# widkyyu/Goal-conditioned-Reinforcement-Learning-with-environmental-and-policy-priors

Measured on AMD Instinct MI355X. Metric: env-steps/sec, higher is better.
Workload: dtype u8

## Files before the change

### goal-conditioned-reinforcement-learning-with-environmental-and-policy-priors_amd/_lib.py

```python
import ctypes as C
import os
import subprocess

_PKG_DIR = os.path.dirname(os.path.abspath(__file__))
LIB_PATH = os.path.join(_PKG_DIR, "libtwoarmy_hip.so")
CSRC_DIR = os.path.join(_PKG_DIR, "csrc")

TW_CELLS = 289
TW_REC_WORDS = 48
TW_DRAW_WORDS = 8
TW_F_AUTORESET = 1
TW_F_POLICY_IDX = 2
TW_F_MATRIX_CODE = 4
TW_F_SLAB_HIPMALLOC = 8

FIELDS = dict(AX=0, AY=1, DIR=2, STEP_COUNT=3, STEP_MOVE=4, PONE=5, PATROL=6, UP1=7, RIGHT2=8, UPD_LONG=9,
              UPD_HORIZ=10, RISK=11, FIRST_ROOM2=12, OBX=13, OBY=16, O1X=19, O1Y=22, O1_VALID=25, O2X=26,
              O2Y=30, O2_VALID=34, GOAL_X=35, GOAL_Y=36, T=37, ERROR=38, MAX_STEPS=39, EPISODES=40,
              LAST_REWARD=41, LAST_TERM=42, LAST_TRUNC=43, WALL_I1=44, WALL_I2=45)

LAUNCH_FIELDS = ("pipelined", "PG", "LAYOUT", "pipe_grid", "E", "FAST", "seq_grid", "T")

ENV_ERRORS = {1: AttributeError, 2: AssertionError, 3: TypeError}

# ... 77 lines not shown
    "mg_obs_goal_direction": (C.c_int, [_vp, _i, _i, _i, _vp, _vp, _i, _i, _vp, _vp, _vp, _vp]),
    "mg_nav_field": (C.c_int, [_vp, _vp, _i, _i, _i, C.c_uint32, _i, _vp, _vp, _i, _vp, _vp, _i, _vp, _i64, _vp, _vp, _vp,
                               _vp]),
    "mg_nav_lookup": (C.c_int, [_vp, _i64, _i, _i, _i, _vp, _i, _vp, _vp]),
    "mg_nav_optimal_moves": (C.c_int, [_vp, _i64, _i, _i, _i, _vp, _vp, _vp, _i, _vp, _vp, _vp]),
    "mg_nav_goal_moves": (C.c_int, [_vp, _vp, _i, _i, _i, C.c_uint32, _i, _vp, _vp, _vp, _i64, _vp, _vp, _vp, _i, _vp, _vp,
                                    _vp]),
    "mg_nav_timed_field": (C.c_int, [_vp, _vp, _i, _i, _i, C.c_uint32, _i, _vp, _i64, _i, _vp, _vp, _i, _vp, _vp, _vp, _i, _vp,
                                     _i64, _vp, _vp, _vp, _vp]),
    "mg_nav_timed_moves": (C.c_int, [_vp, _i64, _i, _i, _i, _i, _vp, _vp, _vp, _i, _vp, _vp, _vp]),
    "mg_nav_timed_goal_moves": (C.c_int, [_vp, _vp, _i, _i, _i, C.c_uint32, _i, _vp, _i64, _i, _vp, _vp, _vp, _i64, _vp, _vp,
                                          _vp, _i, _vp, _vp, _vp]),
    "mg_nav_timed_goal_floods": (C.c_int, [_i, _i, _i]),
    "mg_nav_shape": (C.c_int, [_vp, _i64, _i, _i, _i, _i, _vp, _vp, _vp, _vp, _vp, _vp, _i, _f, _f, _i, _vp, _vp, _vp, _vp]),
    "mg_nav_goal_shape": (C.c_int, [_vp, _vp, _i, _i, _i, C.c_uint32, _i, _vp, _vp, _vp, _vp, _vp, _i64, _vp, _vp, _vp, _vp,
                                    _i, _f, _f, _vp, _vp, _vp, _vp]),
    "mg_nav_timed_goal_shape": (C.c_int, [_vp, _vp, _i, _i, _i, C.c_uint32, _i, _vp, _i64, _i, _vp, _vp, _vp, _vp, _vp, _i64,
                                          _vp, _vp, _vp, _vp, _i, _f, _f, _vp, _vp, _vp, _vp]),
    "mg_nav_timed_goal_shape_floods": (C.c_int, [_i, _i, _i]),
    "mg_nav_ahead": (C.c_int, [_vp, _i64, _i, _i, _i, _i, _vp, _vp, _vp, _i, _i, _vp, _vp, _vp]),
    "mg_nav_goal_ahead": (C.c_int, [_vp, _vp, _i, _i, _i, C.c_uint32, _i, _vp, _vp, _vp, _i64, _vp, _vp, _vp, _i, _i, _vp,
                                    _vp, _vp]),
    "mg_nav_timed_goal_ahead": (C.c_int, [_vp, _vp, _i, _i, _i, C.c_uint32, _i, _vp, _i64, _i, _vp, _vp, _vp, _i64, _vp, _vp,
                                          _vp, _i, _i, _vp, _vp, _vp]),
    "mg_nav_timed_goal_ahead_floods": (C.c_int, [_i, _i, _i]),
    "mg_nav_path_scan": (C.c_int, [_vp, _i64, _i, _i, _i, _i, _vp, _vp, _vp, _vp, _vp, _vp, _i, _vp, _vp, _vp, _vp, _vp, _vp,
                                   _vp, _vp, _vp]),
    "mg_nav_path_summary_workspace": (C.c_int, [_i, _i]),
    "mg_nav_path_summary": (C.c_int, [_vp, _vp, _vp, _vp, _vp, _vp, _i, _i, _vp, _vp, _vp]),
    "ppo_her_relabel": (C.c_int, [_vp, _vp, _vp, _vp, _vp, _vp, _u64, C.c_uint32, C.c_uint32, _i, _i, _i, _vp, _vp, _vp,
                                  _vp, _vp, _vp, _vp, _vp]),
    "ppo_her_relabel_window": (C.c_int, [_vp, _vp, _vp, _vp, _vp, _vp, _u64, C.c_uint32, C.c_uint32, _i, _i, _i, _i, _vp,
                                         _vp, _vp, _vp, _vp, _vp, _vp, _vp]),
    "ppo_lstm_cell": (C.c_int, [_vp, _vp, C.c_longlong, _vp, _vp, _vp, _i, _i, _vp]),
    "ppo_decoder_frames": (C.c_int, [_vp, _i, _vp, _vp, _vp, _vp, _vp, C.c_float, _vp, _vp]),
    "ppo_gather_stack_u8": (C.c_int, [_vp, _i, _vp, _i, _vp, _vp, _vp, _vp, _vp, _i, _vp, _vp, _vp]),
    "ppo_age_scan": (C.c_int, [_vp, _vp, _vp, _i, _i, _vp, _vp]),
    "ppo_episode_scan": (C.c_int, [_vp, _vp, _vp, _i, _i, _vp, _vp, _vp, _vp, _vp]),
    "ppo_episode_summary": (C.c_int, [_vp, _vp, _vp, _vp, _vp, _vp, _i, _i, _i, C.c_double, C.c_double, _vp, _vp, _vp, _vp,
                                      _vp, _vp]),
    "ppo_episode_summary_workspace": (C.c_int, [_i, _i]),
    "ppo_visit_scan": (C.c_int, [_vp, _vp, _vp, _i, _i, _i, _i, _vp, _vp, _vp, _vp]),
    "ppo_visit_carry_words": (C.c_int, [_i, _i, _i]),
    "ppo_visit_hist": (C.c_int, [_vp, _i, _i, _vp, _vp, _vp, _i, _i, _i, _vp, _vp]),
    "ppo_bonus_table_words": (C.c_int, [_i, _i, _i, _i, _i, _i]),
    "ppo_bonus_workspace_bytes": (_i64, [_i, _i, _i, _i, _i, _i]),
    "ppo_bonus_scan": (C.c_int, [_vp, _vp, _vp, C.c_long, C.c_long, _vp, _vp, _i, _i, _i, _i, _i, _i, _i, C.c_double, _vp, _vp,
                                 _vp, _vp, _vp, _vp, _vp]),
    "ppo_bias_relu_nhwc": (C.c_int, [_vp, _vp, _i64, _i, _vp]),
    "ppo_conv1_up4_bias_relu": (C.c_int, [_vp, _i, _i, _vp, _vp, _vp, _vp]),
    "ppo_conv1_up4_bias_relu_c": (C.c_int, [_vp, _i, _i, _i, _vp, _vp, _vp, _vp]),
    "ppo_conv1_up4_bwd_groups": (C.c_int, [_i]),
    "ppo_conv1_up4_bwd": (C.c_int, [_vp, _i, _i, _vp, _vp, _vp, _vp, _vp]),
    "ppo_relu_bwd_bias_grad_nhwc_blocks": (C.c_int, [_i64, _i]),
    "ppo_relu_bwd_bias_grad_nhwc": (C.c_int, [_vp, _vp, _vp, _vp, _i64, _i, _vp]),
})

_lib = None


def exported_symbols():
    return sorted(_SIGS)


def lib():
    global _lib
    if _lib is None:
        if not os.path.exists(LIB_PATH):
            raise TwoarmyLibraryError(
                "%s not built: run `python -c 'import __graft_entry__ as g; g.build()'` "
                "(hipcc --offload-arch=gfx950); there is no CPU fallback" % LIB_PATH)
        import torch
        try:
            h = C.CDLL(LIB_PATH)
        except OSError as ex:
            raise TwoarmyLibraryError("cannot load %s: %s" % (LIB_PATH, ex)) from ex
        for name, (res, args) in _SIGS.items():
            try:
                fn = getattr(h, name)
            except AttributeError as ex:
                raise TwoarmyLibraryError("%s lacks symbol %s" % (LIB_PATH, name)) from ex
            fn.restype, fn.argtypes = res, args
        runtimes = set()
        try:
            with open("/proc/self/maps") as f:
                for line in f:
                    if "libamdhip64" in line:
                        runtimes.add(line.split()[-1])
        except OSError:
            pass
        if h.tw_abi_sizeof_outputs() != C.sizeof(TwOutputs):
            raise TwoarmyLibraryError("struct tw_outputs: the library has %d bytes, the ctypes mirror %d"
                                      % (h.tw_abi_sizeof_outputs(), C.sizeof(TwOutputs)))
        if len(runtimes) > 1:
            raise TwoarmyLibraryError("two HIP runtimes mapped (%s): import torch before loading %s"
                                      % (sorted(runtimes), LIB_PATH))
        _lib = h
    return _lib


def check(rc, what):
    if rc != 0:
        raise TwoarmyLibraryError("%s failed: rc=%d hipError=%d %s" % (
            what, rc, lib().tw_last_hip_error(), lib().tw_last_error_message().decode()))
```

### goal-conditioned-reinforcement-learning-with-environmental-and-policy-priors_amd/csrc/ppo_kernels.hip

```cpp

#include <hip/hip_runtime.h>
#include <float.h>
#include <stdint.h>

#include <type_traits>

#include "launch.h"
#include "philox.h"
#include "twoarmy.h"
#include "twoarmy_ppo.h"

namespace {

constexpr float CAT_EPS = FLT_EPSILON;

template <int A> __device__ __forceinline__ float cat_row(const float *__restrict__ row, float (&p)[A]) {
    float S = 0.f;
#pragma unroll
    for (int k = 0; k < A; ++k) { p[k] = row[k]; S += p[k]; }
    return S;
}
__device__ __forceinline__ float cat_log(float q) { return logf(fminf(fmaxf(q, CAT_EPS), 1.0f - CAT_EPS)); }

template <typename T, int K> __device__ __forceinline__ void block_sum(T (&v)[K], T *lds) {
// ... 131 lines not shown
            float4 acc = bv;
#pragma unroll
            for (int t = 0; t < 4; ++t) {
                const int ty = t >> 1, tx = t & 1;
#pragma unroll
                for (int c = 0; c < F; ++c) acc = fma4(xs[c * 324 + (m + ty) * 18 + n + tx], w[t * F + c], acc);
            }
            dst[((2 * m + py) * 33 + 2 * n + px) * CQ + cq] = relu4(acc);
        }
    }
}

template <int F>
__global__ __launch_bounds__(256) void ppo_conv1_up4_bwd_kernel(const float *__restrict__ frames, const float4 *__restrict__ gy,
                                                                const float4 *__restrict__ y, float4 *__restrict__ gw_part,
                                                                float4 *__restrict__ gb_part, int B) {
    __shared__ float xs[F * 18 * 18];
    __shared__ float4 red[256];
    const int tid = threadIdx.x, cq = tid & 15, slot = tid >> 4;
    const int ph = blockIdx.y, py = ph >> 1, px = ph & 1;
    const int ny = 17 - py, nx = 17 - px;
    float4 acc[4 * F];
#pragma unroll
    for (int k = 0; k < 4 * F; ++k) acc[k] = make_float4(0.f, 0.f, 0.f, 0.f);
    float4 accb = make_float4(0.f, 0.f, 0.f, 0.f);
    for (int b = blockIdx.x; b < B; b += gridDim.x) {
        __syncthreads();
        conv1_stage_frame<F>(xs, frames + (size_t)b * F * 289, tid);
        __syncthreads();
        const size_t base = (size_t)b * 1089 * 16;
        for (int q = slot; q < ny * nx; q += 16) {
            const int m = q / nx, n = q - m * nx;
            const size_t o = base + (size_t)((2 * m + py) * 33 + 2 * n + px) * 16 + cq;
            const float4 g = mask4(gy[o], y[o]);
            add4(accb, g);
#pragma unroll
            for (int t = 0; t < 4; ++t) {
                const int ty = t >> 1, tx = t & 1;
#pragma unroll
                for (int c = 0; c < F; ++c) acc[t * F + c] = fma4(xs[c * 324 + (m + ty) * 18 + n + tx], g, acc[t * F + c]);
            }
        }
    }
    const size_t wbase = ((size_t)blockIdx.x * 4 + ph) * (4 * F) * 16;
#pragma unroll
    for (int k = 0; k <= 4 * F; ++k) {
        __syncthreads();
        red[tid] = k < 4 * F ? acc[k < 4 * F ? k : 0] : accb;
        __syncthreads();
        if (slot == 0) {
            const float4 sum = slot_sum4(red, 16, 16, cq);
            if (k < 4 * F) gw_part[wbase + (size_t)k * 16 + cq] = sum;
            else gb_part[((size_t)blockIdx.x * 4 + ph) * 16 + cq] = sum;
        }
    }
}

constexpr int GT = 64;

template <int GN>
__global__ __launch_bounds__(256) void ppo_gae_kernel(const float *__restrict__ reward, const float *__restrict__ value,
                                                      const float *__restrict__ next_value,
                                                      const uint8_t *__restrict__ done, float gamma, float lambda,
                                                      int use_done_mask, int T, int N, float *__restrict__ adv,
                                                      float *__restrict__ target, float *__restrict__ ret) {
    __shared__ float sd[GT][GN + 1];
    __shared__ float sc[GT][GN + 1];
    __shared__ float carry[GN];
    constexpr int ROWS = 256 / GN;
    const int tid = threadIdx.x, tx = tid % GN, ty = tid / GN;
    const int n = blockIdx.x * GN + tx;
    if (tid < GN) carry[tid] = 0.f;
    const int nchunks = (T + GT - 1) / GT;
    for (int ch = nchunks - 1; ch >= 0; --ch) {
        const int t0 = ch * GT;
        __syncthreads();
        for (int r = ty; r < GT; r += ROWS) {
            const int t = t0 + r;
            float d = 0.f, c = 1.f;
            if (t < T && n < N) {
                const size_t i = (size_t)t * N + n;
                const float cut = (use_done_mask && done[i]) ? 0.f : 1.f;
                const float tv = reward[i] + (gamma * next_value[i]) * cut;
                if (target) target[i] = tv;
                d = tv - value[i];
                c = gamma * lambda * cut;
            }
            sd[r][tx] = d; sc[r][tx] = c;
        }
        __syncthreads();
        const int wave = tid >> 6, lane = tid & 63;
        for (int e = wave * (GN / 4); e < (wave + 1) * (GN / 4); ++e) {
            float d = sd[lane][e], c = sc[lane][e];
#pragma unroll
            for (int off = 1; off < 64; off <<= 1) {
                const float d2 = __shfl_down(d, off), c2 = __shfl_down(c, off);
                if (lane + off < 64 && c != 0.f) { d = fmaf(c, d2, d); c = c * c2; }
            }
            const float a = c != 0.f ? fmaf(c, carry[e], d) : d;
            sd[lane][e] = a;
            const float a0 = __shfl(a, 0);
            if (lane == 0) carry[e] = a0;
        }
        __syncthreads();
        for (int r = ty; r < GT; r += ROWS) {
            const int t = t0 + r;
            if (t < T && n < N) {
                const size_t i = (size_t)t * N + n;
// ... 705 lines not shown
                    const float4 *a = reinterpret_cast<const float4 *>(&a2s[(iy * 33 + ix) * 16]);
                    const float4 *k = reinterpret_cast<const float4 *>(&Ks[(u * 3 + v) * 16]);
#pragma unroll
                    for (int c = 0; c < 4; ++c) {
                        const float4 av = a[c], kv = k[c];
                        acc = fmaf(av.x, kv.x, acc); acc = fmaf(av.y, kv.y, acc);
                        acc = fmaf(av.z, kv.z, acc); acc = fmaf(av.w, kv.w, acc);
                    }
                }
            }
            frames[(size_t)f * 289 + o] = acc;
        }
    }
}

__global__ __launch_bounds__(256) void ppo_lstm_cell_kernel(const float4 *__restrict__ ga, const float4 *__restrict__ gb,
                                                            long long ldb4, const float4 *__restrict__ bias,
                                                            float4 *__restrict__ c, float4 *__restrict__ h, int B, int H4) {
    const int i = blockIdx.x * 256 + threadIdx.x;
    if (i >= B * H4) return;
    const int b = i / H4, j = i - b * H4;
    float4 gi = make_float4(0.f, 0.f, 0.f, 0.f), gf = gi, gg = gi, go = gi;
    if (ga) {
        const float4 *g = ga + (size_t)b * 4 * H4;
        gi = g[j]; gf = g[H4 + j]; gg = g[2 * H4 + j]; go = g[3 * H4 + j];
    }
    auto add4 = [](float4 &a, const float4 &v) { a.x += v.x; a.y += v.y; a.z += v.z; a.w += v.w; };
    if (gb) {
        const float4 *q = gb + (size_t)b * ldb4;
        add4(gi, q[j]); add4(gf, q[H4 + j]); add4(gg, q[2 * H4 + j]); add4(go, q[3 * H4 + j]);
    }
    if (bias) { add4(gi, bias[j]); add4(gf, bias[H4 + j]); add4(gg, bias[2 * H4 + j]); add4(go, bias[3 * H4 + j]); }
    float4 cv = c[i], hv;
    auto sig = [](float x) { return 1.0f / (1.0f + __expf(-x)); };
#define LSTM_LANE(m)                                                                                                      \
    cv.m = sig(gf.m) * cv.m + sig(gi.m) * tanhf(gg.m);                                                                   \
    hv.m = sig(go.m) * tanhf(cv.m);
    LSTM_LANE(x) LSTM_LANE(y) LSTM_LANE(z) LSTM_LANE(w)
#undef LSTM_LANE
    c[i] = cv;
    h[i] = hv;
}

template <typename... P> bool all_set(const P *...p) { return (... && (p != nullptr)); }
template <typename... P> bool aligned16(const P *...p) { return ((... | (uintptr_t)p) & 15u) == 0; }
template <typename... P> bool aligned_natural(const P *...p) { return (... && ((uintptr_t)p % alignof(P) == 0)); }
bool ep_count_ok(int64_t M) { return M < ((int64_t)1 << 40); }
int blocks(int64_t n, int per) { return (int)((n + per - 1) / per); }
int blocks_capped(int64_t n, int per, int cap) { return (int)((n + per - 1) / per < cap ? (n + per - 1) / per : cap); }
int ep_summary_blocks(int64_t M) { return blocks_capped(M, EP_BLOCK_ELEMS, EP_MAX_BLOCKS); }
float4 *f4(float *p) { return reinterpret_cast<float4 *>(p); }
const float4 *f4(const float *p) { return reinterpret_cast<const float4 *>(p); }
template <int V> using int_c = std::integral_constant<int, V>;

#define PPO_ACTION_COUNTS(X) X(5) X(2) X(3) X(4) X(7)
bool ppo_actions_ok(int A) {
#define PPO_IS(V) if (A == V) return true;
    PPO_ACTION_COUNTS(PPO_IS)
#undef PPO_IS
    return false;
}
template <typename Fn> void ppo_with_actions(int A, Fn &&fn) {
    switch (A) {
#define PPO_CASE(V) case V: fn(int_c<V>{}); break;
    PPO_ACTION_COUNTS(PPO_CASE)
#undef PPO_CASE
    }
}

template <typename FT>
int gather_stack(const char *what, const FT *frames, int frame_pitch, const float *pos_frames, int N, const int32_t *k_idx,
                 const int32_t *n_idx, const int32_t *age, const float *init_frame, const float *init_pos, int B,
                 float *out, float *pos_out, void *stream) {
    if (!all_set(frames, k_idx, n_idx, age, init_frame, out) || B <= 0 || frame_pitch < TW_CELLS) return TW_E_ARG;
    if (pos_out && !all_set(pos_frames, init_pos)) return TW_E_ARG;
    hipLaunchKernelGGL(ppo_gather_stack_kernel<FT>, dim3(blocks(B, 4)), dim3(256), 0, (hipStream_t)stream, frames, frame_pitch,
                       pos_frames, N, k_idx, n_idx, age, init_frame, init_pos, B, out, pos_out);
    return tw_launched(what);
}

}

extern "C" {

int ppo_sample(const float *probs, int B, int A, const float *uniforms, uint64_t seed, uint64_t offset,
               int32_t *action, float *logp, void *stream) {
    return ppo_sample_dev(probs, B, A, uniforms, seed, offset, nullptr, action, logp, stream);
}

int ppo_sample_dev(const float *probs, int B, int A, const float *uniforms, uint64_t seed, uint64_t offset,
                   const uint64_t *offset_dev, int32_t *action, float *logp, void *stream) {
    if (!all_set(probs, action, logp) || B <= 0 || !ppo_actions_ok(A)) return TW_E_ARG;
    const uint32_t k0 = (uint32_t)seed, k1 = (uint32_t)(seed >> 32);
    ppo_with_actions(A, [&](auto a) {
        hipLaunchKernelGGL(ppo_sample_kernel<decltype(a)::value>, dim3(blocks(B, 256)), dim3(256), 0, (hipStream_t)stream,
                           probs, B, uniforms, k0, k1, offset, offset_dev, action, logp);
    });
    return tw_launched(__func__);
}

int ppo_gae(const float *reward, const float *value, const float *next_value, const uint8_t *done, float gamma,
            float lambda, int use_done_mask, int T, int N, float *adv, float *target, float *ret, void *stream) {
    if (!all_set(reward, value, next_value) || T <= 0 || N <= 0 || (use_done_mask && !done)) return TW_E_ARG;
    auto launch = [&](auto gn) {
        hipLaunchKernelGGL(ppo_gae_kernel<decltype(gn)::value>, dim3(blocks(N, decltype(gn)::value)), dim3(256), 0,
                           (hipStream_t)stream, reward, value, next_value, done, gamma, lambda, use_done_mask, T, N, adv,
// ... 160 lines not shown
}

int ppo_relu_bwd_bias_grad_nhwc_blocks(int64_t n_pixels, int C) {
    if (n_pixels <= 0 || C <= 0 || (C & 3) || C > 256) return TW_E_ARG;
    return blocks_capped(n_pixels, 512, 4096);
}

int ppo_relu_bwd_bias_grad_nhwc(const float *gy, const float *y, float *gx, float *partial, int64_t n_pixels, int C,
                                void *stream) {
    const int nb = ppo_relu_bwd_bias_grad_nhwc_blocks(n_pixels, C);
    if (nb <= 0 || !all_set(gy, y, gx, partial) || !aligned16(gy, y, gx, partial)) return TW_E_ARG;
    const int ppb = blocks(n_pixels, nb);
    hipLaunchKernelGGL(ppo_relu_bwd_bias_grad_kernel, dim3(nb), dim3(256), 0, (hipStream_t)stream, f4(gy), f4(y), f4(gx),
                       f4(partial), (size_t)n_pixels, C / 4, ppb);
    return tw_launched(__func__);
}

int ppo_conv1_up4_bias_relu(const float *frames, int B, int F, const float *folded_w, const float *bias, float *out,
                            void *stream) {
    return ppo_conv1_up4_bias_relu_c(frames, B, F, 64, folded_w, bias, out, stream);
}

int ppo_conv1_up4_bias_relu_c(const float *frames, int B, int F, int C_out, const float *folded_w, const float *bias,
                              float *out, void *stream) {
    if (!all_set(frames, folded_w, bias, out) || B <= 0 || !aligned16(out, folded_w, bias)) return TW_E_ARG;
    auto launch = [&](auto f, auto cq) {
        hipLaunchKernelGGL((ppo_conv1_up4_kernel<decltype(f)::value, decltype(cq)::value>), dim3(B), dim3(256), 0,
                           (hipStream_t)stream, frames, f4(folded_w), f4(bias), f4(out), B);
    };
    if (F == 4 && C_out == 64) launch(int_c<4>{}, int_c<16>{});
    else if (F == 8 && C_out == 64) launch(int_c<8>{}, int_c<16>{});
    else if (F == 1 && C_out == 16) launch(int_c<1>{}, int_c<4>{});
    else return TW_E_ARG;
    return tw_launched(__func__);
}

int ppo_conv1_up4_bwd_groups(int B) { return B <= 0 ? TW_E_ARG : blocks_capped(B, 1, 256); }

int ppo_conv1_up4_bwd(const float *frames, int B, int F, const float *gy, const float *y, float *gw_partial,
                      float *gb_partial, void *stream) {
    const int groups = ppo_conv1_up4_bwd_groups(B);
    if (groups <= 0 || !all_set(frames, gy, y, gw_partial, gb_partial) || !aligned16(gy, y, gw_partial, gb_partial))
        return TW_E_ARG;
    auto launch = [&](auto f) {
        hipLaunchKernelGGL(ppo_conv1_up4_bwd_kernel<decltype(f)::value>, dim3(groups, 4), dim3(256), 0, (hipStream_t)stream,
                           frames, f4(gy), f4(y), f4(gw_partial), f4(gb_partial), B);
    };
    if (F == 4) launch(int_c<4>{});
    else if (F == 8) launch(int_c<8>{});
    else return TW_E_ARG;
    return tw_launched(__func__);
}

int ppo_decoder_frames(const float *z, int n_frames, const float *w1, const float *b1, const float *w2, const float *b2,
                       const float *kfold, float b3, float *frames, void *stream) {
    if (!all_set(z, w1, b1, w2, b2, kfold, frames) || n_frames <= 0) return TW_E_ARG;
    const int grid = blocks_capped(n_frames, 1, 512);
    hipLaunchKernelGGL(ppo_decoder_frames_kernel, dim3(grid), dim3(256), 0, (hipStream_t)stream, z, n_frames, w1, b1, w2,
                       b2, kfold, b3, frames);
    return tw_launched(__func__);
}

int ppo_lstm_cell(const float *gates_a, const float *gates_b, long long ldb, const float *bias, float *c, float *h, int B,
                  int H, void *stream) {
    if ((!gates_a && !gates_b) || !all_set(c, h) || B <= 0 || H <= 0 || (H & 3) || !aligned16(gates_a, gates_b, bias, c, h))
        return TW_E_ARG;
    if (gates_b && ((ldb & 3) || ldb < 4LL * H)) return TW_E_ARG;
    const long long n = (long long)B * (H / 4);
    if (n > 0x7fffffffLL) return TW_E_ARG;
    hipLaunchKernelGGL(ppo_lstm_cell_kernel, dim3(blocks(n, 256)), dim3(256), 0, (hipStream_t)stream, f4(gates_a),
                       f4(gates_b), ldb / 4, f4(bias), f4(c), f4(h), B, H / 4);
    return tw_launched(__func__);
}

}
```

### goal-conditioned-reinforcement-learning-with-environmental-and-policy-priors_amd/ppo_ops.py

```python
import ctypes as C

import torch

from ._marshal import call as _call, constant as _constant, ptr as _p, query as _query

_CL = torch.channels_last


def _pf(t):
    return _p(t.detach().contiguous(), torch.float32)


def _step_outputs(out, want_steps, T, N, dtypes, device):
    if out is None:
        return tuple(torch.empty((T, N), dtype=d, device=device) if want_steps else None for d in dtypes)
    assert out[0].shape == (T, N) and out[1].shape == (T, N)
    return out


def sample(probs, uniforms=None, seed=0, offset=0, offset_dev=None):
    B, A = probs.shape
    action = torch.empty(B, dtype=torch.int32, device=probs.device)
    logp = torch.empty(B, dtype=torch.float32, device=probs.device)
    _call("ppo_sample_dev", probs, _p(probs, torch.float32), B, A, _p(uniforms, torch.float32), seed, offset,
# ... 195 lines not shown

def bonus_scan(pos, action, reward, state_table=None, action_table=None, scope="env", scale=1.0, width=17, height=17,
               n_actions=7, keep=None, dir=None, dir_ptr=None, bonus_state=None, bonus_action=None, reward_out=None,
               workspace=None):
    T, N = pos.shape[:2]
    assert pos.shape == (T, N, 2)
    for t in (action, reward, keep, bonus_state, bonus_action, reward_out):
        assert t is None or t.shape == (T, N)
    mask = (1 if state_table is not None else 0) | (2 if action_table is not None else 0)
    dp, st, sn = None, 0, 0
    if dir is not None:
        assert dir.shape in ((T, N), (N,))
        dp, st, sn = _p(dir, torch.int32), (N if dir.dim() == 2 else 0), 1
    elif dir_ptr is not None:
        dp, st, sn = C.c_void_p(int(dir_ptr[0])), int(dir_ptr[1]), int(dir_ptr[2])
    if BONUS_SCOPES[scope] == 1:
        need = bonus_workspace_bytes(mask, scope, T, width, height, n_actions)
        if workspace is None:
            workspace = torch.empty(max(1, need // 4), dtype=torch.int32, device=pos.device)
        assert workspace.numel() * 4 >= need
    for kind, tab in (("state", state_table), ("action", action_table)):
        assert tab is None or tab.numel() == bonus_table_words(kind, scope, width, height, n_actions, N)
    _call("ppo_bonus_scan", pos, _p(pos, torch.float32), _p(action, torch.int32), dp, st, sn, _p(reward, torch.float32),
          _p(keep, torch.uint8), T, N, int(width), int(height), int(n_actions), mask, BONUS_SCOPES[scope], float(scale),
          _p(state_table, torch.int32), _p(action_table, torch.int32), _p(bonus_state, torch.float32),
          _p(bonus_action, torch.float32), _p(reward_out, torch.float32), _p(workspace, torch.int32))
    return reward_out


def her_relabel(pos, terminated, truncated, age0, reward, choices=None, seed=0, env_id0=0, step0=0, max_goals=4, skip=0):
    T, N = terminated.shape
    dev = pos.device
    assert pos.shape == (T, N, 2) and pos.is_contiguous() and reward.shape == (T, N)
    if choices is not None:
        assert choices.shape == (T, N, 4) and choices.dtype == torch.int32 and choices.is_contiguous()
    counts = torch.empty(N, dtype=torch.int32, device=dev)
    args = [_p(pos, torch.float32), _p(terminated.contiguous(), torch.uint8), _p(truncated.contiguous(), torch.uint8),
            _p(age0.contiguous(), torch.int32), _p(reward.contiguous(), torch.float32), _p(choices), int(seed),
            int(env_id0), int(step0), T, N, int(max_goals), int(skip)]
    _call("ppo_her_relabel_window", pos, *args, None, _p(counts), None, None, None, None, None)
    incl = torch.cumsum(counts.long(), 0)
    H = int(incl[-1])
    offsets = (incl - counts.long()).contiguous()
    out = dict(t=torch.empty(H, dtype=torch.int32, device=dev), n=torch.empty(H, dtype=torch.int32, device=dev),
               goal=torch.empty((H, 2), dtype=torch.float32, device=dev),
               reward=torch.empty(H, dtype=torch.float32, device=dev), done=torch.empty(H, dtype=torch.uint8, device=dev),
               counts=counts)
    if H:
        _call("ppo_her_relabel_window", pos, *args, _p(offsets), _p(counts), _p(out["t"]), _p(out["n"]), _p(out["goal"]),
              _p(out["reward"]), _p(out["done"]))
    return out


class _ConvBiasReLU(torch.autograd.Function):

    @staticmethod
    def forward(ctx, x, w, b, stride):
        y = torch.ops.aten.convolution(x, w, None, list(stride), [0, 0], [1, 1], False, [0, 0], 1)
        assert y.is_contiguous(memory_format=torch.channels_last), "conv epilogue kernels need channels-last activations"
        B, Cc, H, W = y.shape
        _call("ppo_bias_relu_nhwc", y, _p(y, None, _CL), _pf(b), B * H * W, Cc)
        ctx.save_for_backward(x, w, y)
        ctx.stride = list(stride)
        return y

    @staticmethod
    def backward(ctx, gy):
        x, w, y = ctx.saved_tensors
        gy = gy.contiguous(memory_format=torch.channels_last)
        B, Cc, H, W = y.shape
        npix = B * H * W
        blocks = _query("ppo_relu_bwd_bias_grad_nhwc_blocks", npix, Cc)
        g = torch.empty_like(y)
        partial = torch.empty((blocks, Cc), dtype=torch.float32, device=y.device)
        _call("ppo_relu_bwd_bias_grad_nhwc", y, _p(gy, None, _CL), _p(y, None, _CL), _p(g, None, _CL), _p(partial), npix, Cc)
        gx, gw, _ = torch.ops.aten.convolution_backward(g, x, w, None, ctx.stride, [0, 0], [1, 1], False, [0, 0], 1,
                                                        [bool(ctx.needs_input_grad[0]), True, False])
        return gx, gw, partial.sum(0), None


def conv_bias_relu(x, weight, bias, stride):
    assert x.is_cuda and x.dtype == torch.float32 and x.is_contiguous(memory_format=torch.channels_last)
    return _ConvBiasReLU.apply(x, weight, bias, tuple(stride))


def fold_conv1_weights(w):
    O, F = w.shape[0], w.shape[1]
    w = w.detach().reshape(O, F, 4, 4).float()
    z = torch.zeros_like(w[:, :, 0:1, :])
    rows = torch.stack([torch.cat([w.sum(2, keepdim=True), z], 2),
                        torch.cat([w[:, :, 0:2].sum(2, keepdim=True), w[:, :, 2:4].sum(2, keepdim=True)], 2)], 0)
    zc = torch.zeros_like(rows[..., 0:1])
    cols = torch.stack([torch.cat([rows.sum(-1, keepdim=True), zc], -1),
                        torch.cat([rows[..., 0:2].sum(-1, keepdim=True), rows[..., 2:4].sum(-1, keepdim=True)], -1)], 1)
    return cols.permute(0, 1, 4, 5, 3, 2).contiguous()


@torch.no_grad()
def conv1_up4_bias_relu_infer(frames, weight, bias):
    B, F, _ = frames.shape
    Cout = weight.shape[0]
    y = torch.empty((B, Cout, 33, 33), dtype=torch.float32, device=frames.device, memory_format=torch.channels_last)
    wf = fold_conv1_weights(weight)
    _call("ppo_conv1_up4_bias_relu_c", y, _pf(frames), B, F, Cout, _p(wf), _pf(bias), _p(y, None, _CL))
    return y


class _Conv1Up4(torch.autograd.Function):

    @staticmethod
    def forward(ctx, frames, w, b, wf):
        B, F, _ = frames.shape
        y = torch.empty((B, w.shape[0], 33, 33), dtype=torch.float32, device=frames.device,
                        memory_format=torch.channels_last)
        if wf is None:
            wf = fold_conv1_weights(w)
        fr = frames.contiguous()
        _call("ppo_conv1_up4_bias_relu", y, _p(fr, torch.float32), B, F, _p(wf), _pf(b), _p(y, None, _CL))
        ctx.save_for_backward(fr, w, y)
        return y

    @staticmethod
    def backward(ctx, gy):
        fr, w, y = ctx.saved_tensors
        gy = gy.contiguous(memory_format=torch.channels_last)
        B, F = fr.shape[0], fr.shape[1]
        groups = _query("ppo_conv1_up4_bwd_groups", B)
        gw_part = torch.empty((groups, 2, 2, 2, 2, F, 64), dtype=torch.float32, device=y.device)
        gb_part = torch.empty((groups, 4, 64), dtype=torch.float32, device=y.device)
        _call("ppo_conv1_up4_bwd", y, _p(fr, torch.float32), B, F, _p(gy, None, _CL), _p(y, None, _CL), _p(gw_part),
              _p(gb_part))
        return None, unfold_conv1_grad(gw_part.sum(0)).to(w.dtype), gb_part.sum((0, 1)), None


def unfold_conv1_grad(gwf):
    ty = _constant("conv1_tap_of_row", [[0, 0, 0, 0], [0, 0, 1, 1]], torch.int64, gwf.device)
# ... 43 lines not shown
```

### include/twoarmy_ppo.h

```cpp
#ifndef TWOARMY_PPO_H
#define TWOARMY_PPO_H

#include <stdint.h>

#ifdef __cplusplus
extern "C" {
#endif

int ppo_sample(const float *probs, int B, int A, const float *uniforms, uint64_t seed, uint64_t offset,
               int32_t *action, float *logp, void *stream);
int ppo_sample_dev(const float *probs, int B, int A, const float *uniforms, uint64_t seed, uint64_t offset,
                   const uint64_t *offset_dev, int32_t *action, float *logp, void *stream);

int ppo_gae(const float *reward, const float *value, const float *next_value, const uint8_t *done,
            float gamma, float lambda, int use_done_mask, int T, int N, float *adv, float *target, float *ret,
            void *stream);

int ppo_adv_norm(float *adv, int64_t n, float eps, double *workspace, void *stream);

int ppo_loss_fwd_bwd(const float *probs, const int32_t *action, const float *old_logp, const float *adv,
                     const float *value, const float *target_v, int B, int A, float clip, float ent_coef,
                     float *losses, float *grad_probs, float *grad_value, float *workspace, void *stream);
int ppo_loss_fwd_bwd_masked(const float *probs, const int32_t *action, const float *old_logp, const float *adv,
                            const float *value, const float *target_v, int B, int n_valid, int A, float clip,
// ... 15 lines not shown

int ppo_gather_stack_u8(const uint8_t *frames, int frame_pitch, const float *pos_frames, int N,
                        const int32_t *k_idx, const int32_t *n_idx, const int32_t *age, const float *init_frame,
                        const float *init_pos, int B, float *out, float *pos_out, void *stream);

int ppo_age_scan(const uint8_t *terminated, const uint8_t *truncated, const int32_t *age0, int T, int N,
                 int32_t *age, void *stream);

int ppo_episode_scan(const float *reward, const uint8_t *terminated, const uint8_t *truncated, int T, int N,
                     double *carry_return, int32_t *carry_length, double *ep_return, int32_t *ep_length, void *stream);

int ppo_episode_summary(const double *ep_return, const int32_t *ep_length, const uint8_t *terminated,
                        const uint8_t *truncated, const float *reward, const int32_t *action, int A, int T, int N,
                        double keep, double gain, double *score, double *summary, int64_t *action_hist,
                        int64_t *reward_hist, double *workspace, void *stream);
int ppo_episode_summary_workspace(int T, int N);

int ppo_visit_scan(const float *pos, const uint8_t *terminated, const uint8_t *truncated, int T, int N, int width,
                   int height, uint32_t *carry, uint8_t *first_visit, int32_t *ep_cells, void *stream);
int ppo_visit_carry_words(int width, int height, int N);
int ppo_visit_hist(const float *pos, int T, int N, const uint8_t *mask, const int32_t *t_idx, const int32_t *n_idx, int B,
                   int width, int height, int64_t *counts, void *stream);

int ppo_bonus_table_words(int kind, int scope, int width, int height, int n_actions, int N);
int64_t ppo_bonus_workspace_bytes(int kind_mask, int scope, int T, int width, int height, int n_actions);
int ppo_bonus_scan(const float *pos, const int32_t *action, const int32_t *dir, long dir_stride_t, long dir_stride_n,
                   const float *reward, const uint8_t *keep, int T, int N, int width, int height, int n_actions,
                   int kind_mask, int scope, double scale, void *state_table, void *action_table, float *bonus_state,
                   float *bonus_action, float *reward_out, void *workspace, void *stream);

int ppo_her_relabel(const float *pos, const uint8_t *terminated, const uint8_t *truncated, const int32_t *age0,
                    const float *reward, const int32_t *choices, uint64_t seed, uint32_t env_id0, uint32_t step0, int T,
                    int N, int max_goals, const int64_t *offsets, int32_t *counts, int32_t *out_t, int32_t *out_n,
                    float *out_goal, float *out_reward, uint8_t *out_done, void *stream);
int ppo_her_relabel_window(const float *pos, const uint8_t *terminated, const uint8_t *truncated, const int32_t *age0,
                           const float *reward, const int32_t *choices, uint64_t seed, uint32_t env_id0, uint32_t step0,
                           int T, int N, int max_goals, int skip, const int64_t *offsets, int32_t *counts, int32_t *out_t,
                           int32_t *out_n, float *out_goal, float *out_reward, uint8_t *out_done, void *stream);

int ppo_bias_relu_nhwc(float *y, const float *bias, int64_t n_pixels, int C, void *stream);
int ppo_relu_bwd_bias_grad_nhwc_blocks(int64_t n_pixels, int C);
int ppo_relu_bwd_bias_grad_nhwc(const float *gy, const float *y, float *gx, float *partial, int64_t n_pixels, int C,
                                void *stream);

int ppo_conv1_up4_bias_relu(const float *frames, int B, int F, const float *folded_w, const float *bias, float *out,
                            void *stream);
int ppo_conv1_up4_bias_relu_c(const float *frames, int B, int F, int C_out, const float *folded_w, const float *bias,
                              float *out, void *stream);

int ppo_conv1_up4_bwd_groups(int B);
int ppo_conv1_up4_bwd(const float *frames, int B, int F, const float *gy, const float *y, float *gw_partial,
                      float *gb_partial, void *stream);

int ppo_decoder_frames(const float *z, int n_frames, const float *w1, const float *b1, const float *w2, const float *b2,
                       const float *kfold, float b3, float *frames, void *stream);

int ppo_lstm_cell(const float *gates_a, const float *gates_b, long long ldb, const float *bias, float *c, float *h, int B,
                  int H, void *stream);

#ifdef __cplusplus
}
#endif
#endif
```

Measured before the change: 3.135 billion.

## Add MFMA-based conv2 backward-data kernel replacing aten convolution_backward input grad

Adds a custom HIP kernel for the input gradient of the 64->64 3x3 stride-2 conv on 33x33 inputs. It decomposes the transposed conv into output-parity phases, stages the gradient in LDS and uses fp32 MFMA 32x32x2 instructions with a prepacked weight layout. The aten convolution_backward call now computes only the weight gradient when this path applies. This aims to beat MIOpen's generic backward-data path, at the cost of an extra weight-pack launch per call and a very shape-specific kernel.

Result: no change. 3.135 billion, median of 3 (+0.0%).

```diff
diff --git a/goal-conditioned-reinforcement-learning-with-environmental-and-policy-priors_amd/_lib.py b/goal-conditioned-reinforcement-learning-with-environmental-and-policy-priors_amd/_lib.py
--- a/goal-conditioned-reinforcement-learning-with-environmental-and-policy-priors_amd/_lib.py
+++ b/goal-conditioned-reinforcement-learning-with-environmental-and-policy-priors_amd/_lib.py
@@ -153,6 +153,8 @@
     "ppo_conv1_up4_bias_relu_c": (C.c_int, [_vp, _i, _i, _i, _vp, _vp, _vp, _vp]),
     "ppo_conv1_up4_bwd_groups": (C.c_int, [_i]),
     "ppo_conv1_up4_bwd": (C.c_int, [_vp, _i, _i, _vp, _vp, _vp, _vp, _vp]),
+    "ppo_conv2_bwd_data_workspace": (C.c_int, []),
+    "ppo_conv2_bwd_data": (C.c_int, [_vp, _vp, _i, _vp, _vp, _vp]),
     "ppo_relu_bwd_bias_grad_nhwc_blocks": (C.c_int, [_i64, _i]),
     "ppo_relu_bwd_bias_grad_nhwc": (C.c_int, [_vp, _vp, _vp, _vp, _i64, _i, _vp]),
 })
diff --git a/goal-conditioned-reinforcement-learning-with-environmental-and-policy-priors_amd/csrc/ppo_kernels.hip b/goal-conditioned-reinforcement-learning-with-environmental-and-policy-priors_amd/csrc/ppo_kernels.hip
--- a/goal-conditioned-reinforcement-learning-with-environmental-and-policy-priors_amd/csrc/ppo_kernels.hip
+++ b/goal-conditioned-reinforcement-learning-with-environmental-and-policy-priors_amd/csrc/ppo_kernels.hip
@@ -207,6 +207,114 @@
             const float4 sum = slot_sum4(red, 16, 16, cq);
             if (k < 4 * F) gw_part[wbase + (size_t)k * 16 + cq] = sum;
             else gb_part[((size_t)blockIdx.x * 4 + ph) * 16 + cq] = sum;
+        }
+    }
+}
+
+constexpr int C2_TAP_K[2][2] = {{0, 2}, {1, -1}};
+constexpr int C2_TAP_D[2][2] = {{0, 1}, {0, 0}};
+constexpr int C2_ITEMS[4][6] = {{0, 1, 8, 24, -1, -1}, {2, 3, 9, 25, -1, -1}, {4, 10, 11, 12, 26, -1}, {16, 17, 18, 19, 20, 27}};
+constexpr int C2_PITCH4 = 17;
+typedef float c2_acc_t __attribute__((ext_vector_type(16)));
+
+__global__ __launch_bounds__(256) void ppo_conv2_wpack_kernel(const float *__restrict__ w, float *__restrict__ wp) {
+    const int i = blockIdx.x * 256 + threadIdx.x;
+    const int cr = i & 3, ci = (i >> 2) & 63, cq = (i >> 8) & 15, tap = i >> 12;
+    wp[i] = w[((cq * 4 + cr) * 64 + ci) * 9 + tap];
+}
+
+__device__ __forceinline__ void c2_quad_transpose(float &r0, float &r1, float &r2, float &r3, int lane) {
+    const bool o = lane & 1, p = lane & 2;
+    float s0 = __shfl_xor(o ? r0 : r1, 1), s1 = __shfl_xor(o ? r2 : r3, 1);
+    if (o) { r0 = s0; r2 = s1; } else { r1 = s0; r3 = s1; }
+    s0 = __shfl_xor(p ? r0 : r2, 2), s1 = __shfl_xor(p ? r1 : r3, 2);
+    if (p) { r0 = s0; r1 = s1; } else { r2 = s0; r3 = s1; }
+}
+
+__global__ __launch_bounds__(256, 2) void ppo_conv2_bwd_data_kernel(const float4 *__restrict__ g, const float4 *__restrict__ wp,
+                                                                    float4 *__restrict__ gx) {
+    __shared__ float4 gs[256 * C2_PITCH4];
+    const int tid = threadIdx.x, lane = tid & 63, wave = tid >> 6, r = lane & 31, h = lane >> 5;
+    const float4 *src = g + (size_t)blockIdx.x * 4096;
+#pragma unroll
+    for (int k = 0; k < 16; ++k) {
+        const int i = k * 256 + tid;
+        gs[(i >> 4) * C2_PITCH4 + (i & 15)] = src[i];
+    }
+    __syncthreads();
+    float4 *dst = gx + (size_t)blockIdx.x * (1089 * 16);
+#pragma unroll 1
+    for (int s = 0; s < 6; ++s) {
+        const int item = C2_ITEMS[wave][s];
+        if (item < 0) break;
+        const int py = item >> 4, px = (item >> 3) & 1, pair = item & 7;
+        const int nx = 17 - px, npix = (17 - py) * nx;
+        int my[2], mx[2];
+        bool live[2];
+#pragma unroll
+        for (int u = 0; u < 2; ++u) {
+            const int m = (pair * 2 + u) * 32 + r;
+            live[u] = m < npix;
+            my[u] = m / nx;
+            mx[u] = m - my[u] * nx;
+        }
+        c2_acc_t acc[2][2];
+#pragma unroll
+        for (int u = 0; u < 2; ++u)
+#pragma unroll
+            for (int v = 0; v < 2; ++v)
+#pragma unroll
+                for (int k = 0; k < 16; ++k) acc[u][v][k] = 0.f;
+#pragma unroll 1
+        for (int ty = 0; ty < 2 - py; ++ty) {
+#pragma unroll 1
+            for (int tx = 0; tx < 2 - px; ++tx) {
+                const int tap = C2_TAP_K[py][ty] * 3 + C2_TAP_K[px][tx];
+                int aoff[2];
+                bool ok[2];
+#pragma unroll
+                for (int u = 0; u < 2; ++u) {
+                    const int oy = my[u] - C2_TAP_D[py][ty], ox = mx[u] - C2_TAP_D[px][tx];
+                    ok[u] = live[u] && (unsigned)oy < 16u && (unsigned)ox < 16u;
+                    aoff[u] = ok[u] ? (oy * 16 + ox) * C2_PITCH4 + h : h;
+                }
+                const float4 *wt = wp + ((tap * 16 + h) * 64 + r);
+#pragma unroll
+                for (int c = 0; c < 8; ++c) {
+                    float4 a[2], bq[2];
+#pragma unroll
+                    for (int u = 0; u < 2; ++u) {
+                        a[u] = gs[aoff[u] + 2 * c];
+                        if (!ok[u]) a[u] = make_float4(0.f, 0.f, 0.f, 0.f);
+                    }
+#pragma unroll
+                    for (int v = 0; v < 2; ++v) bq[v] = wt[c * 128 + v * 32];
+#pragma unroll
+                    for (int u = 0; u < 2; ++u)
+#pragma unroll
+                        for (int v = 0; v < 2; ++v) {
+                            acc[u][v] = __builtin_amdgcn_mfma_f32_32x32x2f32(a[u].x, bq[v].x, acc[u][v], 0, 0, 0);
+                            acc[u][v] = __builtin_amdgcn_mfma_f32_32x32x2f32(a[u].y, bq[v].y, acc[u][v], 0, 0, 0);
+                            acc[u][v] = __builtin_amdgcn_mfma_f32_32x32x2f32(a[u].z, bq[v].z, acc[u][v], 0, 0, 0);
+                            acc[u][v] = __builtin_amdgcn_mfma_f32_32x32x2f32(a[u].w, bq[v].w, acc[u][v], 0, 0, 0);
+                        }
+                }
+            }
+        }
+#pragma unroll
+        for (int u = 0; u < 2; ++u) {
+#pragma unroll
+            for (int q = 0; q < 4; ++q) {
+                const int m = (pair * 2 + u) * 32 + 8 * q + 4 * h + (r & 3);
+                const int oy = m / nx, ox = m - oy * nx;
+                const int pix = (2 * oy + py) * 33 + 2 * ox + px;
+#pragma unroll
+                for (int v = 0; v < 2; ++v) {
+                    float c0 = acc[u][v][4 * q], c1 = acc[u][v][4 * q + 1], c2 = acc[u][v][4 * q + 2], c3 = acc[u][v][4 * q + 3];
+                    c2_quad_transpose(c0, c1, c2, c3, lane);
+                    if (m < npix) dst[pix * 16 + 8 * v + (r >> 2)] = make_float4(c0, c1, c2, c3);
+                }
+            }
         }
     }
 }
@@ -1286,6 +1394,16 @@
     return tw_launched(__func__);
 }
 
+int ppo_conv2_bwd_data_workspace(void) { return 9 * 64 * 64; }
+
+int ppo_conv2_bwd_data(const float *g, const float *w, int B, float *wpack, float *gx, void *launch_stream) {
+    if (!all_set(g, w, wpack, gx) || B <= 0 || !aligned16(g, w, wpack, gx)) return TW_E_ARG;
+    const hipStream_t st = (hipStream_t)launch_stream;
+    hipLaunchKernelGGL(ppo_conv2_wpack_kernel, dim3(9 * 64 * 64 / 256), dim3(256), 0, st, w, wpack);
+    hipLaunchKernelGGL(ppo_conv2_bwd_data_kernel, dim3(B), dim3(256), 0, st, f4(g), f4(wpack), f4(gx));
+    return tw_launched(__func__);
+}
+
 int ppo_decoder_frames(const float *z, int n_frames, const float *w1, const float *b1, const float *w2, const float *b2,
                        const float *kfold, float b3, float *frames, void *stream) {
     if (!all_set(z, w1, b1, w2, b2, kfold, frames) || n_frames <= 0) return TW_E_ARG;
diff --git a/goal-conditioned-reinforcement-learning-with-environmental-and-policy-priors_amd/ppo_ops.py b/goal-conditioned-reinforcement-learning-with-environmental-and-policy-priors_amd/ppo_ops.py
--- a/goal-conditioned-reinforcement-learning-with-environmental-and-policy-priors_amd/ppo_ops.py
+++ b/goal-conditioned-reinforcement-learning-with-environmental-and-policy-priors_amd/ppo_ops.py
@@ -274,13 +274,16 @@
 class _ConvBiasReLU(torch.autograd.Function):
 
     @staticmethod
-    def forward(ctx, x, w, b, stride):
+    def forward(ctx, x, w, b, stride, conv2_kernel=True):
         y = torch.ops.aten.convolution(x, w, None, list(stride), [0, 0], [1, 1], False, [0, 0], 1)
         assert y.is_contiguous(memory_format=torch.channels_last), "conv epilogue kernels need channels-last activations"
         B, Cc, H, W = y.shape
         _call("ppo_bias_relu_nhwc", y, _p(y, None, _CL), _pf(b), B * H * W, Cc)
         ctx.save_for_backward(x, w, y)
         ctx.stride = list(stride)
+        ctx.conv2 = bool(conv2_kernel and tuple(x.shape[1:]) == (64, 33, 33) and tuple(w.shape) == (64, 64, 3, 3)
+                         and ctx.stride == [2, 2] and w.dtype == torch.float32
+                         and x.is_contiguous(memory_format=torch.channels_last))
         return y
 
     @staticmethod
@@ -293,14 +296,27 @@
         g = torch.empty_like(y)
         partial = torch.empty((blocks, Cc), dtype=torch.float32, device=y.device)
         _call("ppo_relu_bwd_bias_grad_nhwc", y, _p(gy, None, _CL), _p(y, None, _CL), _p(g, None, _CL), _p(partial), npix, Cc)
+        own = ctx.conv2 and ctx.needs_input_grad[0]
         gx, gw, _ = torch.ops.aten.convolution_backward(g, x, w, None, ctx.stride, [0, 0], [1, 1], False, [0, 0], 1,
-                                                        [bool(ctx.needs_input_grad[0]), True, False])
-        return gx, gw, partial.sum(0), None
-
-
-def conv_bias_relu(x, weight, bias, stride):
+                                                        [bool(ctx.needs_input_grad[0]) and not own, True, False])
+        if own:
+            gx = conv2_bwd_data(g, w)
+        return gx, gw, partial.sum(0), None, None
+
+
+def conv2_bwd_data(g, w):
+    assert tuple(g.shape[1:]) == (64, 16, 16) and tuple(w.shape) == (64, 64, 3, 3)
+    B = g.shape[0]
+    gx = torch.empty((B, 64, 33, 33), dtype=torch.float32, device=g.device, memory_format=torch.channels_last)
+    wpack = torch.empty(_query("ppo_conv2_bwd_data_workspace"), dtype=torch.float32, device=g.device)
+    wc = w.detach().contiguous()
+    _call("ppo_conv2_bwd_data", g, _p(g, torch.float32, _CL), _p(wc, torch.float32), B, _p(wpack), _p(gx, None, _CL))
+    return gx
+
+
+def conv_bias_relu(x, weight, bias, stride, _conv2_kernel=True):
     assert x.is_cuda and x.dtype == torch.float32 and x.is_contiguous(memory_format=torch.channels_last)
-    return _ConvBiasReLU.apply(x, weight, bias, tuple(stride))
+    return _ConvBiasReLU.apply(x, weight, bias, tuple(stride), _conv2_kernel)
 
 
 def fold_conv1_weights(w):
diff --git a/include/twoarmy_ppo.h b/include/twoarmy_ppo.h
--- a/include/twoarmy_ppo.h
+++ b/include/twoarmy_ppo.h
@@ -91,6 +91,9 @@
 int ppo_conv1_up4_bwd(const float *frames, int B, int F, const float *gy, const float *y, float *gw_partial,
                       float *gb_partial, void *stream);
 
+int ppo_conv2_bwd_data_workspace(void);
+int ppo_conv2_bwd_data(const float *g, const float *w, int B, float *wpack, float *gx, void *launch_stream);
+
 int ppo_decoder_frames(const float *z, int n_frames, const float *w1, const float *b1, const float *w2, const float *b2,
                        const float *kfold, float b3, float *frames, void *stream);
 
```

## Add MFMA weight-gradient kernel for conv2/conv3 NHWC backward

Applied to the files above, without the earlier changes.

Adds a custom HIP weight-gradient (wrw) kernel for the two stride-2 NHWC conv layers. It uses fp32 MFMA 32x32x2 with register-prefetched LDS staging and a row ring buffer, and the bias gradient is fused into the same pass. Per-slice partials are reduced by a second kernel. The ConvBiasReLU backward now calls it in place of the weight half of aten convolution_backward, keeping aten only for the input gradient. This aims to beat MIOpen's wrw path, at the cost of an extra partial buffer and a reduction launch.

New measurement: 2.772 billion before, 2.758 billion after. No clear change (-0.5%).

```diff
diff --git a/goal-conditioned-reinforcement-learning-with-environmental-and-policy-priors_amd/_lib.py b/goal-conditioned-reinforcement-learning-with-environmental-and-policy-priors_amd/_lib.py
--- a/goal-conditioned-reinforcement-learning-with-environmental-and-policy-priors_amd/_lib.py
+++ b/goal-conditioned-reinforcement-learning-with-environmental-and-policy-priors_amd/_lib.py
@@ -155,6 +155,8 @@
     "ppo_conv1_up4_bwd": (C.c_int, [_vp, _i, _i, _vp, _vp, _vp, _vp, _vp]),
     "ppo_relu_bwd_bias_grad_nhwc_blocks": (C.c_int, [_i64, _i]),
     "ppo_relu_bwd_bias_grad_nhwc": (C.c_int, [_vp, _vp, _vp, _vp, _i64, _i, _vp]),
+    "ppo_conv_wrw_slices": (C.c_int, [_i, _i]),
+    "ppo_conv_wrw_nhwc": (C.c_int, [_vp, _vp, _i, _i, _i, _i, _i, _vp, _vp, _vp, _vp, _vp]),
 })
 
 _lib = None
diff --git a/goal-conditioned-reinforcement-learning-with-environmental-and-policy-priors_amd/csrc/ppo_kernels.hip b/goal-conditioned-reinforcement-learning-with-environmental-and-policy-priors_amd/csrc/ppo_kernels.hip
--- a/goal-conditioned-reinforcement-learning-with-environmental-and-policy-priors_amd/csrc/ppo_kernels.hip
+++ b/goal-conditioned-reinforcement-learning-with-environmental-and-policy-priors_amd/csrc/ppo_kernels.hip
@@ -209,6 +209,136 @@
             else gb_part[((size_t)blockIdx.x * 4 + ph) * 16 + cq] = sum;
         }
     }
+}
+
+typedef float wrw_acc_t __attribute__((ext_vector_type(16)));
+typedef float wrw_f4_t __attribute__((ext_vector_type(4)));
+constexpr int WRW_C = 64;
+struct wrw_conv2 {
+    static constexpr int O = 64, KS = 3, HI = 33, WI = 33, HO = 16, WO = 16, NKY = 3, OYS = 1, MB = 1, SLOTS = 3, NEW = 3;
+    static constexpr int CAP = 512;
+    static constexpr bool RING = true;
+};
+struct wrw_conv3 {
+    static constexpr int O = 128, KS = 4, HI = 16, WI = 16, HO = 7, WO = 7, NKY = 1, OYS = 7, MB = 2, SLOTS = 7, NEW = 7;
+    static constexpr int CAP = 256;
+    static constexpr bool RING = false;
+};
+
+template <typename L>
+__global__ __launch_bounds__(256) void ppo_conv_wrw_kernel(const float4 *__restrict__ g, const float4 *__restrict__ x,
+                                                           float *__restrict__ partial, float4 *__restrict__ partial_b,
+                                                           int B, int per) {
+    constexpr int O = L::O, O4 = O / 4, PU = L::OYS * L::WO, KSTEPS = (PU + 1) / 2, UPS = L::HO / L::OYS;
+    constexpr int ROW4 = L::WI * (WRW_C / 4);
+    constexpr int XJ = (L::NEW * ROW4 + 255) / 256, GJ = (PU * O4 + 255) / 256;
+    constexpr int NT = L::NKY * L::KS, N = L::KS * L::KS * WRW_C;
+    __shared__ float4 xs4[L::SLOTS * ROW4];
+    __shared__ float4 gs4[2 * KSTEPS * O4];
+    __shared__ float4 red[256];
+    const float *xs = reinterpret_cast<const float *>(xs4), *gs = reinterpret_cast<const float *>(gs4);
+    const int tid = threadIdx.x, lane = tid & 63, w = tid >> 6, half = lane >> 5, l32 = lane & 31;
+    const int mgrp = w & 1, chalf = w >> 1, ky0 = blockIdx.y * L::NKY;
+    const int b0 = blockIdx.x * per, nb = (B - b0 < per ? B - b0 : per), units = nb * UPS;
+    if (PU & 1) for (int i = tid; i < O4; i += 256) gs4[PU * O4 + i] = make_float4(0.f, 0.f, 0.f, 0.f);
+
+    wrw_acc_t acc[L::MB][NT];
+#pragma unroll
+    for (int i = 0; i < L::MB; ++i)
+#pragma unroll
+        for (int t = 0; t < NT; ++t)
+#pragma unroll
+            for (int r = 0; r < 16; ++r) acc[i][t][r] = 0.f;
+    float4 accb = make_float4(0.f, 0.f, 0.f, 0.f);
+    wrw_f4_t xr[XJ], gr[GJ];
+
+    auto fetch = [&](int u) __attribute__((always_inline)) {
+        const int b = b0 + u / UPS, oy0 = (u % UPS) * L::OYS;
+        const int first = L::RING ? (oy0 == 0 ? 0 : 2 * oy0 + 1) : ky0, count = L::RING ? (oy0 == 0 ? 3 : 2) : L::NEW;
+        const wrw_f4_t *xb = reinterpret_cast<const wrw_f4_t *>(x) + (size_t)b * L::HI * ROW4;
+        const wrw_f4_t *gb = reinterpret_cast<const wrw_f4_t *>(g) + ((size_t)b * L::HO + oy0) * L::WO * O4;
+#pragma unroll
+        for (int j = 0; j < XJ; ++j) {
+            const int i = tid + j * 256, rj = i / ROW4;
+            xr[j] = i < count * ROW4 ? xb[(first + (L::RING ? rj : 2 * rj)) * ROW4 + (i - rj * ROW4)] : xb[0];
+        }
+#pragma unroll
+        for (int j = 0; j < GJ; ++j) gr[j] = gb[tid + j * 256 < PU * O4 ? tid + j * 256 : 0];
+    };
+    auto stage = [&](int u) __attribute__((always_inline)) {
+        const int oy0 = (u % UPS) * L::OYS;
+        const int first = L::RING ? (oy0 == 0 ? 0 : 2 * oy0 + 1) : 0, count = L::RING ? (oy0 == 0 ? 3 : 2) : L::NEW;
+#pragma unroll
+        for (int j = 0; j < XJ; ++j) {
+            const int i = tid + j * 256, rj = i / ROW4;
+            if (i < count * ROW4) xs4[(L::RING ? (first + rj) % 3 : rj) * ROW4 + (i - rj * ROW4)] = make_float4(xr[j].x, xr[j].y, xr[j].z, xr[j].w);
+        }
+#pragma unroll
+        for (int j = 0; j < GJ; ++j)
+            if (tid + j * 256 < PU * O4) {
+                const float4 v = make_float4(gr[j].x, gr[j].y, gr[j].z, gr[j].w);
+                gs4[tid + j * 256] = v;
+                add4(accb, v);
+            }
+    };
+
+    if (units > 0) fetch(0);
+    for (int u = 0; u < units; ++u) {
+        __syncthreads();
+        stage(u);
+        __syncthreads();
+        if (u + 1 < units) fetch(u + 1);
+        const int ring0 = (2 * ((u % UPS) * L::OYS)) % 3;
+#pragma unroll
+        for (int k = 0; k < KSTEPS; ++k) {
+            const int p = 2 * k + half, pc = p < PU ? p : PU - 1;
+            const int oyl = pc / L::WO, ox = pc - oyl * L::WO;
+            float a[L::MB];
+#pragma unroll
+            for (int i = 0; i < L::MB; ++i) a[i] = gs[p * O + (mgrp * L::MB + i) * 32 + l32];
+#pragma unroll
+            for (int kyl = 0; kyl < L::NKY; ++kyl) {
+                const int slot = L::RING ? (ring0 + kyl) % 3 : oyl * L::NKY + kyl;
+#pragma unroll
+                for (int kx = 0; kx < L::KS; ++kx) {
+                    const float bv = xs[(slot * L::WI + 2 * ox + kx) * WRW_C + chalf * 32 + l32];
+#pragma unroll
+                    for (int i = 0; i < L::MB; ++i)
+                        acc[i][kyl * L::KS + kx] = __builtin_amdgcn_mfma_f32_32x32x2f32(a[i], bv, acc[i][kyl * L::KS + kx], 0, 0, 0);
+                }
+            }
+        }
+    }
+
+    float *out = partial + (size_t)blockIdx.x * O * N;
+#pragma unroll
+    for (int i = 0; i < L::MB; ++i)
+#pragma unroll
+        for (int t = 0; t < NT; ++t)
+#pragma unroll
+            for (int r = 0; r < 16; ++r) {
+                const int o = (mgrp * L::MB + i) * 32 + (r & 3) + 8 * (r >> 2) + 4 * half;
+                out[o * N + (ky0 * L::KS + t) * WRW_C + chalf * 32 + l32] = acc[i][t][r];
+            }
+    __syncthreads();
+    red[tid] = accb;
+    __syncthreads();
+    if (blockIdx.y == 0 && tid < O4) partial_b[(size_t)blockIdx.x * O4 + tid] = slot_sum4(red, 256 / O4, O4, tid);
+}
+
+__global__ __launch_bounds__(256) void ppo_conv_wrw_sum_kernel(const float4 *__restrict__ partial,
+                                                               const float4 *__restrict__ partial_b, int S, int n4, int o4,
+                                                               float4 *__restrict__ gw, float4 *__restrict__ gb) {
+    const int i = blockIdx.x * 256 + threadIdx.x;
+    if (i >= n4 + o4) return;
+    const bool bias = i >= n4;
+    const float4 *src = bias ? partial_b + (i - n4) : partial + i;
+    const size_t stride = bias ? o4 : n4;
+    float4 sum = src[0];
+#pragma unroll 8
+    for (int s = 1; s < S; ++s) add4(sum, src[s * stride]);
+    if (bias) gb[i - n4] = sum;
+    else gw[i] = sum;
 }
 
 constexpr int GT = 64;
@@ -1020,6 +1150,7 @@
 float4 *f4(float *p) { return reinterpret_cast<float4 *>(p); }
 const float4 *f4(const float *p) { return reinterpret_cast<const float4 *>(p); }
 template <int V> using int_c = std::integral_constant<int, V>;
+int wrw_per(int B, int cap) { return blocks(B, cap) < 2 ? 2 : blocks(B, cap); }
 
 #define PPO_ACTION_COUNTS(X) X(5) X(2) X(3) X(4) X(7)
 bool ppo_actions_ok(int A) {
@@ -1286,6 +1417,28 @@
     return tw_launched(__func__);
 }
 
+int ppo_conv_wrw_slices(int B, int layer) {
+    return B <= 0 || (layer != 2 && layer != 3) ? TW_E_ARG : blocks(B, wrw_per(B, layer == 2 ? wrw_conv2::CAP : wrw_conv3::CAP));
+}
+
+int ppo_conv_wrw_nhwc(const float *g, const float *x, int B, int C, int O, int k, int H_in, float *partial,
+                      float *partial_b, float *gw, float *gb, void *launch_stream) {
+    const int layer = (C == 64 && O == 64 && k == 3 && H_in == 33) ? 2 : (C == 64 && O == 128 && k == 4 && H_in == 16) ? 3 : 0;
+    if (!layer || B <= 0 || !all_set(g, x, partial, partial_b, gw, gb) || !aligned16(g, x, partial, partial_b, gw, gb))
+        return TW_E_ARG;
+    auto launch = [&](auto l) {
+        using L = decltype(l);
+        if ((int64_t)B * L::HO * L::WO > 0x7fffffffLL) return TW_E_ARG;
+        const int S = ppo_conv_wrw_slices(B, layer), n4 = L::O * L::KS * L::KS * WRW_C / 4, o4 = L::O / 4;
+        hipLaunchKernelGGL(ppo_conv_wrw_kernel<L>, dim3(S, L::KS / L::NKY), dim3(256), 0, (hipStream_t)launch_stream, f4(g),
+                           f4(x), partial, f4(partial_b), B, wrw_per(B, L::CAP));
+        hipLaunchKernelGGL(ppo_conv_wrw_sum_kernel, dim3(blocks(n4 + o4, 256)), dim3(256), 0, (hipStream_t)launch_stream,
+                           f4(partial), f4(partial_b), S, n4, o4, f4(gw), f4(gb));
+        return tw_launched("ppo_conv_wrw_nhwc");
+    };
+    return layer == 2 ? launch(wrw_conv2{}) : launch(wrw_conv3{});
+}
+
 int ppo_decoder_frames(const float *z, int n_frames, const float *w1, const float *b1, const float *w2, const float *b2,
                        const float *kfold, float b3, float *frames, void *stream) {
     if (!all_set(z, w1, b1, w2, b2, kfold, frames) || n_frames <= 0) return TW_E_ARG;
diff --git a/goal-conditioned-reinforcement-learning-with-environmental-and-policy-priors_amd/ppo_ops.py b/goal-conditioned-reinforcement-learning-with-environmental-and-policy-priors_amd/ppo_ops.py
--- a/goal-conditioned-reinforcement-learning-with-environmental-and-policy-priors_amd/ppo_ops.py
+++ b/goal-conditioned-reinforcement-learning-with-environmental-and-policy-priors_amd/ppo_ops.py
@@ -271,6 +271,34 @@
     return out
 
 
+WRW_LAYERS = {(64, 64, 3, 33): 2, (64, 128, 4, 16): 3}
+
+
+def conv_wrw_layer(g, x, w, stride=(2, 2)):
+    if not all(t.is_cuda and t.dtype == torch.float32 and t.dim() == 4 and t.is_contiguous(memory_format=_CL)
+               for t in (g, x, w)) or tuple(stride) != (2, 2):
+        return 0
+    O, Cin, k, k2 = w.shape
+    H = x.shape[2]
+    Ho = (H - k) // 2 + 1
+    ok = k == k2 and x.shape[1:] == (Cin, H, H) and g.shape == (x.shape[0], O, Ho, Ho)
+    return WRW_LAYERS.get((Cin, O, k, H), 0) if ok else 0
+
+
+def conv_wrw(g, x, w, workspace=None):
+    B, (O, Cin, k, _) = x.shape[0], w.shape
+    S = _query("ppo_conv_wrw_slices", B, WRW_LAYERS.get((Cin, O, k, x.shape[2]), 0))
+    part, part_b = workspace if workspace is not None else (
+        torch.empty((S, O, k, k, Cin), dtype=torch.float32, device=x.device),
+        torch.empty((S, O), dtype=torch.float32, device=x.device))
+    assert part.numel() >= S * O * k * k * Cin and part_b.numel() >= S * O
+    gw = torch.empty_like(w)
+    gb = torch.empty(O, dtype=torch.float32, device=x.device)
+    _call("ppo_conv_wrw_nhwc", x, _p(g, torch.float32, _CL), _p(x, torch.float32, _CL), B, Cin, O, k, x.shape[2],
+          _p(part, torch.float32), _p(part_b, torch.float32), _p(gw, torch.float32, _CL), _p(gb))
+    return gw, gb
+
+
 class _ConvBiasReLU(torch.autograd.Function):
 
     @staticmethod
@@ -293,8 +321,13 @@
         g = torch.empty_like(y)
         partial = torch.empty((blocks, Cc), dtype=torch.float32, device=y.device)
         _call("ppo_relu_bwd_bias_grad_nhwc", y, _p(gy, None, _CL), _p(y, None, _CL), _p(g, None, _CL), _p(partial), npix, Cc)
-        gx, gw, _ = torch.ops.aten.convolution_backward(g, x, w, None, ctx.stride, [0, 0], [1, 1], False, [0, 0], 1,
-                                                        [bool(ctx.needs_input_grad[0]), True, False])
+        own, need_gx = bool(conv_wrw_layer(g, x, w, ctx.stride)), bool(ctx.needs_input_grad[0])
+        gx = gw = None
+        if need_gx or not own:
+            gx, gw, _ = torch.ops.aten.convolution_backward(g, x, w, None, ctx.stride, [0, 0], [1, 1], False, [0, 0], 1,
+                                                            [need_gx, not own, False])
+        if own:
+            return (gx,) + conv_wrw(g, x, w) + (None,)
         return gx, gw, partial.sum(0), None
 
 
diff --git a/include/twoarmy_ppo.h b/include/twoarmy_ppo.h
--- a/include/twoarmy_ppo.h
+++ b/include/twoarmy_ppo.h
@@ -91,6 +91,10 @@
 int ppo_conv1_up4_bwd(const float *frames, int B, int F, const float *gy, const float *y, float *gw_partial,
                       float *gb_partial, void *stream);
 
+int ppo_conv_wrw_slices(int B, int layer);
+int ppo_conv_wrw_nhwc(const float *g, const float *x, int B, int C, int O, int k, int H_in, float *partial,
+                      float *partial_b, float *gw, float *gb, void *launch_stream);
+
 int ppo_decoder_frames(const float *z, int n_frames, const float *w1, const float *b1, const float *w2, const float *b2,
                        const float *kfold, float b3, float *frames, void *stream);
 
```
